# HydrogenSulfate/LFT

Hardware: AMD Instinct MI355X
Metric: LF patches/sec (5x5 angRes, 32x32 LR, 4xSR) (higher is better)
Workload: dtype bf16; 1 GPU; LFT 5x5 angRes 4xSR inference, batch=4 per GPU, 32x32 LR patches; global_batch=4, parallelism=dp1 (independent shards), streams_per_gpu=1, hip_graph=True, steps_in_flight=2

## Files before the change

### lft_amd/_lib.py

```python
from __future__ import annotations

import ctypes
import os
import subprocess
from ctypes import POINTER, c_char_p, c_float, c_int, c_longlong, c_size_t, c_void_p

HERE = os.path.dirname(os.path.abspath(__file__))
CSRC = os.path.join(HERE, "csrc")
LIB_PATH = os.environ.get("LFT_LIB_PATH") or os.path.join(HERE, "liblft_hip.so")
SOURCES = ["lft_api.hip", "lft_common.cuh", "lft_kernels_a.cuh", "lft_kernels_b.cuh", "lft_train.cuh", "lft_train_host.cuh", "lft_metrics.cuh", "lft_prepare.cuh"]
ABI_VERSION = 5
STATUS_NONFINITE = 1001

PREC_F32, PREC_BF16, PREC_F16 = 0, 1, 2
MATH_F32, MATH_BF16X3, MATH_BF16X6 = 0, 1, 2
NUM_PARAMS = 78

_lib = None


class LftError(RuntimeError):
    pass


# ... 73 lines not shown
                                     c_int, POINTER(c_float), POINTER(c_char_p), POINTER(c_int)]),
    "lft_kernel_time": (c_int, [c_char_p, c_void_p, c_void_p, c_int, c_int, c_int, c_int, c_int, c_int, c_int, c_void_p, POINTER(c_float)]),
    "lft_bicubic_fwd": (c_int, [c_void_p, c_void_p, c_int, c_int, c_int, c_int, c_int, c_void_p]),
    "lft_init_features_fwd": (c_int, [c_void_p, c_void_p, c_void_p, c_void_p, c_int, c_int, c_int, c_int, c_int, c_int, c_void_p]),
    "lft_ang_block_fwd": (c_int, [c_void_p, c_int, c_void_p, c_void_p, c_int, c_int, c_int, c_int, c_int, c_int, c_void_p]),
    "lft_spa_block_fwd": (c_int, [c_void_p, c_int, c_void_p, c_void_p, c_void_p, c_void_p, c_int, c_int, c_int, c_int, c_int, c_int, c_void_p]),
    "lft_upsample_fwd": (c_int, [c_void_p, c_void_p, c_void_p, c_void_p, c_void_p, c_int, c_int, c_int, c_int, c_int, c_int, c_void_p]),
    "lft_scene_counts": (c_int, [c_int, c_int, c_int, c_int, POINTER(c_int), POINTER(c_int)]),
    "lft_scene_divide": (c_int, [c_void_p, c_void_p, c_int, c_int, c_int, c_int, c_int, c_void_p]),
    "lft_scene_integrate": (c_int, [c_void_p, c_void_p, c_int, c_int, c_int, c_int, c_int, c_int, c_void_p]),
    "lft_train_tape_bytes": (c_int, [c_int, c_int, c_int, c_int, c_int, POINTER(c_size_t)]),
    "lft_train_grad_floats": (c_int, [c_int, POINTER(c_size_t)]),
    "lft_train_tape_offset": (c_int, [c_char_p, c_int, c_int, c_int, c_int, c_int, POINTER(c_size_t)]),
    "lft_train_forward": (c_int, [POINTER(c_void_p), c_int, c_void_p, c_void_p, c_void_p, c_int, c_int, c_int, c_int, c_int, c_int, c_void_p]),
    "lft_train_backward": (c_int, [POINTER(c_void_p), c_int, c_void_p, c_void_p, c_void_p, c_void_p, c_int, c_int, c_int, c_int, c_int, c_int, c_void_p]),
    "lft_train_backward_input": (c_int, [POINTER(c_void_p), c_int, c_void_p, c_void_p, c_void_p, c_void_p, c_void_p,
                                         c_int, c_int, c_int, c_int, c_int, c_int, c_void_p]),
    "lft_lr_grad_bwd": (c_int, [c_void_p, c_void_p, c_void_p, c_void_p, c_int, c_int, c_int, c_int, c_int, c_void_p]),
    "lft_train_backward_buckets": (c_int, [POINTER(c_void_p), c_int, c_void_p, c_void_p, c_void_p, c_void_p, c_int, c_int, c_int, c_int, c_int, c_int,
                                           c_void_p, c_void_p, c_void_p]),
    "lft_train_block_backward": (c_int, [POINTER(c_void_p), c_int, c_void_p, c_void_p, c_int, c_int, c_void_p, c_void_p, c_void_p,
                                         c_int, c_int, c_int, c_int, c_int, c_int, c_void_p]),
    "lft_train_grad_bucket": (c_int, [c_int, c_int, POINTER(c_size_t), POINTER(c_size_t)]),
    "lft_train_step_profiled": (c_int, [POINTER(c_void_p), c_int, c_void_p, c_void_p, c_void_p, c_void_p, c_void_p, c_int, c_int, c_int, c_int, c_int, c_int,
                                        c_void_p, c_int, POINTER(c_float), POINTER(c_char_p), POINTER(c_int)]),
    "lft_l1_loss": (c_int, [c_void_p, c_void_p, c_longlong, c_void_p, c_float, c_void_p, c_void_p, c_void_p]),
    "lft_adam_step": (c_int, [c_void_p, c_void_p, c_void_p, c_void_p, c_longlong, c_float, c_float, c_float, c_float, c_int, c_float, c_float, c_void_p]),
    "lft_view_metrics_scratch_bytes": (c_int, [c_int, c_int, c_int, c_int, POINTER(c_size_t)]),
    "lft_view_metrics": (c_int, [c_void_p, c_void_p, c_int, c_int, c_int, c_int, c_float, c_void_p, c_void_p, c_void_p, c_void_p]),
    "lft_lf_prepare": (c_int, [c_void_p, c_int, c_int, c_int, c_int, c_int, c_int, POINTER(c_longlong), c_int, c_int,
                               POINTER(c_int), c_int, c_int, c_int, c_void_p, c_void_p, c_int, c_void_p, c_void_p, c_int,
                               c_void_p, c_void_p, c_void_p]),
    "lft_mfma_selftest": (c_int, [c_void_p, c_void_p, c_void_p, c_void_p, c_void_p, c_int, c_void_p]),
}
EXPORTS = tuple(_SIGS)
TEST_EXPORTS = ("lft_mfma_selftest",)
BLOCK_UPSAMPLE, BLOCK_SPA, BLOCK_ANG, BLOCK_INIT = 0, 1, 2, 3
LF_UINT8, LF_FLOAT32, LF_FLOAT64 = 0, 1, 2
GRAD_BUCKETS = 3
BUCKET_FN = ctypes.CFUNCTYPE(c_int, c_void_p, c_int, c_size_t, c_size_t)


def lib() -> ctypes.CDLL:
    global _lib
    if _lib is None:
        if not os.path.exists(LIB_PATH):
            raise LftError(f"{LIB_PATH} is missing: the HIP extension has not been built "
                           "(run __graft_entry__.build()); there is no CPU fallback")
        L = ctypes.CDLL(LIB_PATH)
        L.lft_version.restype, L.lft_version.argtypes = c_int, []
        got = L.lft_version()
        if got != ABI_VERSION:
            raise LftError(f"{LIB_PATH} reports ABI version {got}, this binding needs {ABI_VERSION}: rebuild it (__graft_entry__.build())")
        for name, (res, args) in _SIGS.items():
            fn = getattr(L, name)
            fn.restype, fn.argtypes = res, args
        _lib = L
    return _lib


def check(rc: int, what: str) -> None:
    if rc != 0:
        msg = lib().lft_last_error()
        raise LftError(f"{what} failed (code {rc}): {msg.decode() if msg else ''}")


def packed_bytes(A, h, w, s, prec) -> int:
    n = c_size_t(0)
    check(lib().lft_packed_bytes(A, h, w, s, prec, ctypes.byref(n)), "lft_packed_bytes")
    return n.value


def workspace_bytes(B, A, h, w, s, prec) -> int:
    n = c_size_t(0)
    check(lib().lft_workspace_bytes(B, A, h, w, s, prec, ctypes.byref(n)), "lft_workspace_bytes")
    return n.value
```

### lft_amd/csrc/lft_api.hip

```cpp
#include "../../include/lft_hip.h"
#include "../../include/lft_hip_test.h"
#include <hip/hip_runtime.h>
#include <stdint.h>

#include <cstdarg>
#include <cstdio>
#include <cmath>
#include <set>
#include <string>
#include <algorithm>
#include <type_traits>
#include <utility>
#include <vector>

#ifndef LFT_TU
#define LFT_TU 0
#endif

namespace {
#include "lft_kernels_a.cuh"
#include "lft_kernels_b.cuh"
#include "lft_metrics.cuh"
#include "lft_prepare.cuh"
#include "lft_train.cuh"
// ... 78 lines not shown

template <auto... Vs, typename V, typename F> int dispatch(V v, F&& f) {
    int rc = 0;
    if (((v == Vs && ((rc = f(std::integral_constant<decltype(Vs), Vs>{})), true)) || ...)) return rc;
    return fail(LFT_ERR_ARG, "internal: no kernel variant for %d", (int)v);
}
template <int V> using int_c = std::integral_constant<int, V>;
template <typename F> int by_prec(int prec, F&& f) {
    if (prec == LFT_PREC_F32) return f(float{});
    if (prec == LFT_PREC_BF16) return f(bf16_t{});
    return f(f16_t{});
}
inline size_t align256(size_t x) { return (x + 255) & ~(size_t)255; }

struct Dims {
    int B, A, V, h, w, hw, s, gp, gt, nchunk;
    long long ntok;
};

int make_dims(int B, int A, int h, int w, int s, int prec, Dims* d) {
    if (prec != LFT_PREC_F32 && prec != LFT_PREC_BF16 && prec != LFT_PREC_F16)
        return fail(LFT_ERR_ARG, "prec must be LFT_PREC_F32, LFT_PREC_BF16 or LFT_PREC_F16, got %d", prec);
    if (B < 1 || A < 1 || h < 1 || w < 1) return fail(LFT_ERR_SHAPE, "B, A, h, w must be positive (B=%d A=%d h=%d w=%d)", B, A, h, w);
    if (s != 2 && s != 4) return fail(LFT_ERR_SHAPE, "scale factor must be 2 or 4, got %d", s);
    if (A * A > 128) return fail(LFT_ERR_UNSUPPORTED, "angRes %d (A*A=%d views > 128) is not implemented in this build", A, A * A);
    if ((long long)B * A * A * h * w > (1LL << 27)) return fail(LFT_ERR_SHAPE, "too many tokens");
    d->B = B; d->A = A; d->V = A * A; d->h = h; d->w = w; d->hw = h * w; d->s = s;
    d->gp = (s + 2) * (s + 2); d->gt = (d->gp + 31) / 32; d->nchunk = 2 * s * s;
    d->ntok = (long long)B * d->V * d->hw;
    return 0;
}

constexpr int kFragsConv = 72, kFragsAng = 64, kFragsSpa1 = 240, kFragsSpa1NoQ = 208, kFragsSpa2 = 176;
inline int frags_up(const Dims& d) { return d.nchunk * (4 + 2 * d.gt); }

struct PackedLayout {
    size_t conv0_w, ln_ang[kLayers], ln_spa[kLayers], ang_pe, petok[kLayers], spa_pe_img;
    size_t s_conv[3], s_ang[kLayers], s_spa1[kLayers], s_spa2[kLayers], s_up, total;
};

PackedLayout packed_layout(const Dims& d, int prec) {
    const size_t esz = prec == LFT_PREC_F32 ? 4 : 2, fragb = 64 * 8 * esz;
    PackedLayout L;
    size_t o = 0;
    auto take = [&](size_t bytes) { size_t r = o; o = align256(o + bytes); return r; };
    L.conv0_w = take(576 * 4);
    for (int l = 0; l < kLayers; ++l) { L.ln_ang[l] = take(256 * 4); L.ln_spa[l] = take(512 * 4); }
    L.ang_pe = take((size_t)((d.V + 31) / 32) * 2048 * 4);
    for (int l = 0; l < kLayers; ++l) L.petok[l] = take((size_t)((d.hw + 32 * kNwSpa1 - 1) / (32 * kNwSpa1)) * kNwSpa1 * 4096 * esz);
    L.spa_pe_img = take((size_t)d.hw * 64 * esz);
    for (int i = 0; i < 3; ++i) L.s_conv[i] = take(kFragsConv * fragb);
    for (int l = 0; l < kLayers; ++l) {
        L.s_ang[l] = take(kFragsAng * fragb);
        L.s_spa1[l] = take(kFragsSpa1 * fragb);
        L.s_spa2[l] = take(kFragsSpa2 * fragb);
    }
    L.s_up = take((size_t)frags_up(d) * fragb);
    L.total = o;
    return L;
}

struct WorkLayout {
    size_t x0, feat, xa, xb, tok, q, k, v, o, g, status, total;
};
WorkLayout work_layout(const Dims& d, int prec) {
    const size_t esz = prec == LFT_PREC_F32 ? 4 : 2;
    WorkLayout W;
// ... 119 lines not shown
            std::vector<PackOp> ops;
            ops.push_back(lin_op(q[12], 0, 64, 64, 0, 4, 1, kAngScale));
            ops.push_back(lin_op(q[12], 64, 64, 64, 0, 4, 1, 1.0f));
            ops.push_back(lin_op(q[12], 128, 64, 64, 0, 4, 1, 1.0f));
            ops.push_back(lin_op(q[13], 0, 64, 64, 0, 4, 1, 1.0f));
            ops.push_back(lin_op(q[16], 0, 128, 64, 0, 4, 1, 1.0f));
            ops.push_back(lin_op(q[17], 0, 64, 128, 0, 8, 1, 1.0f));
            if ((rc = run_pack<T>(ops, at<T>(packed, L.s_ang[l]), kFragsAng, st))) return rc;
        }
        {
            std::vector<PackOp> ops;
            conv_ops(ops, q[0], 128);
            ops.push_back(lin_op(q[3], 256, 128, 128, 0, 8, 1, 1.0f));
            ops.push_back(lin_op(q[3], 128, 128, 128, 0, 8, 1, 1.0f));
            ops.push_back(lin_op(q[3], 0, 128, 128, 0, 8, 1, kSpaScale));
            if ((rc = run_pack<T>(ops, at<T>(packed, L.s_spa1[l]), kFragsSpa1, st))) return rc;
        }
        {
            std::vector<PackOp> ops;
            ops.push_back(lin_op(q[4], 0, 128, 128, 0, 8, (sizeof(T) == 2 && tok_lane_major<T>(d)) ? 1 : 0, 1.0f));
            for (int c = 0; c < 4; ++c) {
                ops.push_back(lin_op(q[7], 64 * c, 64, 128, 0, 8, 1, 1.0f));
                ops.push_back(lin_op(q[8], 0, 128, 256, 64 * c, 4, 1, 1.0f));
            }
            ops.push_back(lin_op(q[9], 0, 64, 128, 0, 8, 1, 1.0f));
            if ((rc = run_pack<T>(ops, at<T>(packed, L.s_spa2[l]), kFragsSpa2, st))) return rc;
        }
        if ((rc = launch_spa1<T, true>((unsigned)((d.hw + 32 * kNwSpa1 - 1) / (32 * kNwSpa1)), at<T>(packed, L.spa_pe_img), at<T>(packed, L.s_spa1[l]), nullptr, nullptr,
                                       nullptr, nullptr, nullptr, nullptr, at<T>(packed, L.petok[l]), 1, d, st, nullptr))) return rc;
        LFT_LAUNCH_OK("k_spa1<pe>");
    }
    {
        std::vector<PackOp> ops;
        for (int c = 0; c < d.nchunk; ++c) {
            ops.push_back(lin_op(P[76], 32 * c, 32, 64, 0, 4, 1, 1.0f));
            PackOp m = lin_op(P[77], 0, d.gp, 0, 32 * c, 2, 1, 1.0f);
            m.kind = 1; m.s = d.s; m.ntiles = d.gt;
            ops.push_back(m);
        }
        if ((rc = run_pack<T>(ops, at<T>(packed, L.s_up), frags_up(d), st))) return rc;
    }
    return 0;
}

void launch_assemble(const float* lr, const float* g, float* out, int B, int A, int h, int w, int s, hipStream_t st, int gld = 0, unsigned* status = nullptr) {
    const dim3 tg((unsigned)((A * w + 7) / 8) * (unsigned)((A * h + 7) / 8) * (unsigned)B);
    if (!gld) gld = (s + 2) * (s + 2);
    if (s == 2) k_assemble_t<2><<<tg, 256, 0, st>>>(lr, g, out, B, A, h, w, gld, status);
    else k_assemble_t<4><<<tg, 256, 0, st>>>(lr, g, out, B, A, h, w, gld, status);
}

template <typename T>
int init_features(const void* packed, const PackedLayout& L, const float* lr, T* x0, T* ta, T* tb, T* feat, const Dims& d, hipStream_t st) {
    const int nimg = d.B * d.V, nwg = nimg * ((d.hw + 32 * kNwConv - 1) / (32 * kNwConv));
    const size_t lds = lds_conv64<T>(d.w);
    int rc;
    if ((rc = allow_lds(k_conv64<T, false>, lds, "k_conv64"))) return rc;
    if ((rc = allow_lds(k_conv64<T, true>, lds, "k_conv64"))) return rc;
    k_conv0<T><<<dim3((unsigned)((d.hw + kConv0Tok - 1) / kConv0Tok), (unsigned)nimg), 256, 0, st>>>(lr, at<float>(packed, L.conv0_w), x0, d.B, d.A, d.h, d.w);
    LFT_LAUNCH_OK("k_conv0");
    k_conv64<T, false><<<nwg, 64 * kNwConv, lds, st>>>(x0, ta, nullptr, at<T>(packed, L.s_conv[0]), nimg, d.h, d.w);
    LFT_LAUNCH_OK("k_conv64");
    k_conv64<T, false><<<nwg, 64 * kNwConv, lds, st>>>(ta, tb, nullptr, at<T>(packed, L.s_conv[1]), nimg, d.h, d.w);
    LFT_LAUNCH_OK("k_conv64");
    k_conv64<T, true><<<nwg, 64 * kNwConv, lds, st>>>(tb, feat, x0, at<T>(packed, L.s_conv[2]), nimg, d.h, d.w);
    LFT_LAUNCH_OK("k_conv64");
    return 0;
}
template <typename T, int CT, int LL>
int ang_multi(const void* packed, const PackedLayout& L, int l, const T* in, T* out, const Dims& d, hipStream_t st, unsigned* status) {
    constexpr bool WLDS = sizeof(T) == 2;
    constexpr int NG = (sizeof(T) == 2 && CT <= 3) ? 2 : 1;
    constexpr size_t FB = 1024 * FragInfo<T>::PIECES;
    const size_t lds = (WLDS ? 64 * FB : 0) + 1024 + (size_t)NG * CT * 8 * FB + (size_t)NG * CT * TileIO<2, T>::BYTES;
    const int npix = d.B * d.hw;
    int rc;
    const unsigned grid = std::min<unsigned>(blocks_for(npix, NG), 256u * (unsigned)std::max<size_t>(1, kMaxLds / lds));
    if ((rc = allow_lds(k_ang_multi<T, CT, WLDS, NG, LL>, lds, "k_ang_multi"))) return rc;
    k_ang_multi<T, CT, WLDS, NG, LL><<<grid, 64 * CT * NG, lds, st>>>(in, out, at<T>(packed, L.s_ang[l]), at<float>(packed, L.ln_ang[l]),
                                                                     at<float>(packed, L.ang_pe), d.V, d.hw, npix, status);
    LFT_LAUNCH_OK("k_ang");
    return 0;
}
template <typename T>
int ang_block(const void* packed, const PackedLayout& L, int l, const T* in, T* out, const Dims& d, hipStream_t st, unsigned* status = nullptr) {
    auto multi = [&](auto CT, auto LL) { return ang_multi<T, CT, LL>(packed, L, l, in, out, d, st, status); };
    if (d.V > 100) return multi(int_c<4>{}, int_c<13>{});
    if (d.V > 96) return multi(int_c<4>{}, int_c<9>{});
    if (d.V > 64) return multi(int_c<3>{}, int_c<9>{});
    if (d.V == 64) return multi(int_c<2>{}, int_c<16>{});
    if (d.V > 32) return multi(int_c<2>{}, int_c<9>{});
    const int npix = d.B * d.hw;
    const size_t lds = lds_ang<T>();
    int rc;
    const unsigned grid = std::min<unsigned>(blocks_for(npix, 4), 256u * (unsigned)std::max<size_t>(1, kMaxLds / lds));
// ... 213 lines not shown
int lft_kernel_time(const char* kernel, const void* packed, void* workspace, int B, int A, int h, int w, int s, int prec, int reps,
                    void* stream, float* ms_out) {
    Dims d; int rc;
    if (!kernel || !packed || !workspace || !ms_out || reps < 1) return fail(LFT_ERR_ARG, "bad argument");
    if ((rc = make_dims(B, A, h, w, s, prec, &d))) return rc;
    hipStream_t st = static_cast<hipStream_t>(stream);
    return by_prec(prec, [&](auto t) { using T = decltype(t); return kernel_time_impl<T>(kernel, packed, workspace, d, prec, reps, st, ms_out); });
}

int lft_bicubic_fwd(const float* lr, float* out, int B, int A, int h, int w, int s, void* stream) {
    Dims d; int rc;
    if (!lr || !out) return fail(LFT_ERR_ARG, "null pointer");
    if ((rc = make_dims(B, A, h, w, s, LFT_PREC_F32, &d))) return rc;
    const dim3 grid((unsigned)((A * w * s + 255) / 256), (unsigned)(A * h * s), (unsigned)B);
    k_bicubic<<<grid, 256, 0, static_cast<hipStream_t>(stream)>>>(lr, out, B, A, h, w, s);
    LFT_LAUNCH_OK("k_bicubic");
    return 0;
}

int lft_init_features_fwd(const void* packed, const float* lr, void* act_out, void* workspace, int B, int A, int h, int w, int s,
                          int prec, void* stream) {
    Dims d; int rc;
    if (!packed || !lr || !act_out || !workspace) return fail(LFT_ERR_ARG, "null pointer");
    if ((rc = make_dims(B, A, h, w, s, prec, &d))) return rc;
    const PackedLayout L = packed_layout(d, prec);
    const WorkLayout W = work_layout(d, prec);
    hipStream_t st = static_cast<hipStream_t>(stream);
    return by_prec(prec, [&](auto t) {
        using T = decltype(t);
        return init_features<T>(packed, L, lr, at<T>(workspace, W.x0), at<T>(workspace, W.xa), at<T>(workspace, W.xb), static_cast<T*>(act_out), d, st);
    });
}

int lft_ang_block_fwd(const void* packed, int layer, const void* act_in, void* act_out, int B, int A, int h, int w, int s, int prec,
                      void* stream) {
    Dims d; int rc;
    if (!packed || !act_in || !act_out) return fail(LFT_ERR_ARG, "null pointer");
    if (layer < 0 || layer >= kLayers) return fail(LFT_ERR_ARG, "layer %d out of range", layer);
    if ((rc = make_dims(B, A, h, w, s, prec, &d))) return rc;
    const PackedLayout L = packed_layout(d, prec);
    hipStream_t st = static_cast<hipStream_t>(stream);
    return by_prec(prec, [&](auto t) {
        using T = decltype(t);
        return ang_block<T>(packed, L, layer, static_cast<const T*>(act_in), static_cast<T*>(act_out), d, st);
    });
}

int lft_spa_block_fwd(const void* packed, int layer, const void* act_in, const void* skip, void* act_out, void* workspace, int B, int A,
                      int h, int w, int s, int prec, void* stream) {
    Dims d; int rc;
    if (!packed || !act_in || !act_out || !workspace) return fail(LFT_ERR_ARG, "null pointer");
    if (layer < 0 || layer >= kLayers) return fail(LFT_ERR_ARG, "layer %d out of range", layer);
    if ((rc = make_dims(B, A, h, w, s, prec, &d))) return rc;
    const PackedLayout L = packed_layout(d, prec);
    const WorkLayout W = work_layout(d, prec);
    hipStream_t st = static_cast<hipStream_t>(stream);
    return by_prec(prec, [&](auto t) {
        using T = decltype(t);
        return spa_block<T>(packed, L, layer, static_cast<const T*>(act_in), static_cast<const T*>(skip), static_cast<T*>(act_out), workspace, W, d, st);
    });
}

int lft_upsample_fwd(const void* packed, const void* act_in, const float* lr, float* out, void* workspace, int B, int A, int h, int w,
                     int s, int prec, void* stream) {
    Dims d; int rc;
    if (!packed || !act_in || !lr || !out || !workspace) return fail(LFT_ERR_ARG, "null pointer");
// ... 29 lines not shown
    return 0;
}
int lft_scene_counts(int h0, int w0, int patch, int stride, int* num_u, int* num_v) {
    if (!num_u || !num_v) return fail(LFT_ERR_ARG, "null pointer");
    return scene_counts(h0, w0, patch, stride, num_u, num_v);
}
int lft_scene_divide(const float* scene, float* patches, int A, int h0, int w0, int patch, int stride, void* stream) {
    int nu, nv, rc;
    if (!scene || !patches || A < 1) return fail(LFT_ERR_ARG, "bad argument");
    if ((rc = scene_counts(h0, w0, patch, stride, &nu, &nv))) return rc;
    const dim3 grid((unsigned)((A * patch + 255) / 256), (unsigned)(A * patch), (unsigned)(nu * nv));
    k_scene_divide<<<grid, 256, 0, static_cast<hipStream_t>(stream)>>>(scene, patches, A, h0, w0, patch, stride, nv);
    LFT_LAUNCH_OK("k_scene_divide");
    return 0;
}
int lft_scene_integrate(const float* sr_patches, float* sr_scene, int A, int h0, int w0, int patch, int stride, int s, void* stream) {
    int nu, nv, rc;
    if (!sr_patches || !sr_scene || A < 1 || s < 1) return fail(LFT_ERR_ARG, "bad argument");
    if ((rc = scene_counts(h0, w0, patch, stride, &nu, &nv))) return rc;
    const dim3 grid((unsigned)((A * w0 * s + 255) / 256), (unsigned)(A * h0 * s));
    k_scene_integrate<<<grid, 256, 0, static_cast<hipStream_t>(stream)>>>(sr_patches, sr_scene, A, patch * s, stride * s, h0 * s, w0 * s, nv);
    LFT_LAUNCH_OK("k_scene_integrate");
    return 0;
}

int lft_mfma_selftest(const float* Am, const float* Bm, const float* W2, float* C, float* D, int prec, void* stream) {
    if (!Am || !Bm || !W2 || !C || !D) return fail(LFT_ERR_ARG, "null pointer");
    hipStream_t st = static_cast<hipStream_t>(stream);
    if (prec == LFT_PREC_F32) k_selftest<float><<<1, 64, 0, st>>>(Am, Bm, W2, C, D);
    else if (prec == LFT_PREC_BF16) k_selftest<bf16_t><<<1, 64, 0, st>>>(Am, Bm, W2, C, D);
    else if (prec == LFT_PREC_F16) k_selftest<f16_t><<<1, 64, 0, st>>>(Am, Bm, W2, C, D);
    else return fail(LFT_ERR_ARG, "bad prec %d", prec);
    LFT_LAUNCH_OK("k_selftest");
    return 0;
}

int lft_view_metrics_scratch_bytes(int B, int A, int h, int w, size_t* out_bytes) {
    if (!out_bytes || B < 1 || A < 1 || h < 1 || w < 1) return fail(LFT_ERR_ARG, "bad argument");
    const size_t ntiles = (size_t)((h + kMetTile - 1) / kMetTile) * ((w + kMetTile - 1) / kMetTile);
    *out_bytes = (size_t)B * A * A * ntiles * 3 * sizeof(double);
    return 0;
}
int lft_view_metrics(const float* label, const float* out, int B, int A, int h, int w, float ssim_range, float* psnr, float* ssim,
                     void* scratch, void* stream) {
    if (!label || !out || !psnr || !ssim || !scratch || B < 1 || A < 1) return fail(LFT_ERR_ARG, "bad argument");
    if (h < 11 || w < 11) return fail(LFT_ERR_SHAPE, "views of %dx%d are smaller than the 11x11 SSIM window", h, w);
    hipStream_t st = static_cast<hipStream_t>(stream);
    const int ntiles = ((h + kMetTile - 1) / kMetTile) * ((w + kMetTile - 1) / kMetTile), nviews = B * A * A;
    const double C1 = (0.01 * ssim_range) * (0.01 * ssim_range), C2 = (0.03 * ssim_range) * (0.03 * ssim_range);
    k_view_metrics<<<dim3((unsigned)ntiles, (unsigned)nviews), 256, 0, st>>>(label, out, static_cast<double*>(scratch), A, h, w, C1, C2);
    LFT_LAUNCH_OK("k_view_metrics");
    k_view_metrics_final<<<blocks_for(nviews, 64), 64, 0, st>>>(static_cast<const double*>(scratch), nviews, ntiles, h, w, psnr, ssim);
    LFT_LAUNCH_OK("k_view_metrics_final");
    return 0;
}
int lft_lf_prepare(const void* lf, int lf_class, int U, int V, int H, int W, int C, const long long* strides, int A, int s,
                   const int* crops, int n_crops, int crop_h, int crop_w, const double* weights_h, const int* indices_h, int taps_h,
                   const double* weights_w, const int* indices_w, int taps_w, float* hr, float* lr, void* stream) {
    if (!lf || !strides || !crops || !weights_h || !indices_h || !weights_w || !indices_w || !hr || !lr)
        return fail(LFT_ERR_ARG, "lft_lf_prepare: null pointer");
    if (lf_class != LFT_LF_UINT8 && lf_class != LFT_LF_FLOAT32 && lf_class != LFT_LF_FLOAT64)
        return fail(LFT_ERR_ARG, "lft_lf_prepare: light-field class must be LFT_LF_UINT8, LFT_LF_FLOAT32 or LFT_LF_FLOAT64, got %d", lf_class);
    if (U < 1 || V < 1 || H < 1 || W < 1 || C < 3)
        return fail(LFT_ERR_ARG, "lft_lf_prepare: light field [%d,%d,%d,%d,%d] needs positive sizes and at least 3 channels", U, V, H, W, C);
    for (int i = 0; i < 5; ++i)
        if (strides[i] < 0) return fail(LFT_ERR_ARG, "lft_lf_prepare: stride %d is negative (%lld)", i, strides[i]);
// ... 182 lines not shown
```

### lft_amd/csrc/lft_kernels_a.cuh

```cuda
#pragma once
#include "lft_common.cuh"

struct PackOp {
    const float* src;
    int kind, row0, nrows, ntiles, ld, kmul, kadd, k0, ksteps, kmap, frag0, s;
    float scale;
    int order;
};
__host__ __device__ __forceinline__ int wfrag_index(int OT, int KS, int ot, int ks) {
    const int g = ot >> 2, G = OT - 4 * g < 4 ? OT - 4 * g : 4;
    return 4 * g * KS + ks * G + (ot & 3);
}
__host__ __device__ __forceinline__ void wfrag_coords(int OT, int KS, int lf, int order, int& nt, int& ks) {
    if (!order) { nt = lf / KS; ks = lf % KS; return; }
    const int gl = (OT - 1) >> 2, g = lf / (4 * KS) < gl ? lf / (4 * KS) : gl, G = OT - 4 * g < 4 ? OT - 4 * g : 4, rem = lf - 4 * g * KS;
    ks = rem / G; nt = 4 * g + rem % G;
}
constexpr int LFT_PACK_MAXOPS = 40;
struct PackArgs {
    int nops;
    PackOp op[LFT_PACK_MAXOPS];
};

LFT_DEV float upm_entry(const float* __restrict__ w3, int n, int kk, int s) {
    const int I = n / (s + 2) - 1, J = n % (s + 2) - 1;
    const int c = kk / (s * s), i = (kk / s) % s, j = kk % s;
    const int dy = i - I, dx = j - J;
    if (dy < -1 || dy > 1 || dx < -1 || dx > 1) return 0.0f;
    return w3[c * 9 + (dy + 1) * 3 + (dx + 1)];
}

template <typename T>
__global__ __launch_bounds__(64) void k_pack(PackArgs args, T* __restrict__ dst) {
    const int f = blockIdx.x, lane = threadIdx.x, r = lane & 31, h = lane >> 5;
    int oi = 0;
    for (int i = 0; i < args.nops; ++i)
        if (f >= args.op[i].frag0) oi = i;
    const PackOp& op = args.op[oi];
    int nt, ks;
    wfrag_coords(op.ntiles, op.ksteps, f - op.frag0, op.order, nt, ks);
    const int n = 32 * nt + r;
#pragma unroll
    for (int j = 0; j < 8; ++j) {
        const int kk = op.k0 + 16 * ks + (op.kmap ? 8 * (j >> 2) + 4 * h + (j & 3) : 8 * h + j);
        float v = 0.0f;
        if (n < op.nrows) {
            if (op.kind == 0) v = op.scale * op.src[(size_t)(op.row0 + n) * op.ld + kk * op.kmul + op.kadd];
            else if (op.kind == 1) v = upm_entry(op.src, n, kk, op.s);
            else v = kk < (op.s + 2) * (op.s + 2) ? upm_entry(op.src, kk, n, op.s) : 0.0f;
        }
        if constexpr (sizeof(T) == 4) dst[(((size_t)f * 2 + (j >> 2)) * 64 + lane) * 4 + (j & 3)] = (T)v;
        else dst[((size_t)f * 64 + lane) * 8 + j] = (T)v;
    }
}

LFT_DEV float pe_value(int l, int c) {
    const int m = c & 31;
    const float g = (float)pow(10000.0, (double)(2 * m) / 64.0);
    const float p = (float)l / g;
    return (c < 32) ? (float)sin((double)p) : (float)cos((double)p);
}
template <typename T>
__global__ void k_pe_tables(float* __restrict__ ang_pe, T* __restrict__ spa_img, int V, int h, int w) {
    const int idx = blockIdx.x * blockDim.x + threadIdx.x;
    const int ntile = (V + 31) / 32;
    if (idx < ntile * 2048) {
        const int e = idx & 7, lane = (idx >> 3) & 63, k = (idx >> 9) & 3, ct = idx >> 11;
        const int view = ct * 32 + (lane & 31), nt = k >> 1, g = 2 * (k & 1) + (e >> 2);
        const int ch = 32 * nt + 8 * g + 4 * (lane >> 5) + (e & 3);
        ang_pe[idx] = view < V ? pe_value(view, ch) : 0.0f;
    }
    if (idx < h * w * 64) {
        const int p = idx >> 6, c = idx & 63;
        spa_img[idx] = (T)((pe_value(p / w, c) + pe_value(p % w, c)) / 2.0f);
    }
}
__global__ void k_copy_f32(const float* __restrict__ src, float* __restrict__ dst, int n) {
    const int i = blockIdx.x * blockDim.x + threadIdx.x;
    if (i < n) dst[i] = src[i];
}

// ... 96 lines not shown

constexpr int kConvZeroRow = 256;
LFT_DEV void clear_zero_row(char* zero_row) {
    if (threadIdx.x < kConvZeroRow / 16) store_raw16(zero_row + threadIdx.x * 16, raw16{0u, 0u, 0u, 0u});
}
template <int NT, typename T, int NW, typename Ring>
LFT_DEV void conv3x3_tile(const char* lds_in, const char* zero_row, int tl, int y, int x, bool ok, int h, int w, int hh,
                          Ring& ring, f32x16 (&acc)[NT]) {
    using CI = ConvIn<T, NW>;
    static_assert(CI::ROW_BYTES <= kConvZeroRow, "zero row too short");
#pragma unroll
    for (int tap = 0; tap < 9; ++tap) {
        const int dy = tap / 3 - 1, dx = tap % 3 - 1;
        const int yy = y + dy, xx = x + dx;
        const bool inb = ok && yy >= 0 && yy < h && xx >= 0 && xx < w;
        const int slot = tl + w + 1 + dy * w + dx;
        const char* row = inb ? lds_in + slot * CI::ROW_BYTES : zero_row;
        const int sw = inb ? CI::swz(slot) : 0;
#pragma unroll
        for (int ks = 0; ks < 4; ++ks) {
            Frag<T> b;
            if constexpr (sizeof(T) == 2) {
                b.v = __builtin_bit_cast(typename H16<T>::v8, load_raw16(row + (((2 * ks + hh) ^ sw) * 16)));
            } else {
                b.lo = __builtin_bit_cast(f32x4, load_raw16(row + (((4 * ks + 2 * hh) ^ sw) * 16)));
                b.hi = __builtin_bit_cast(f32x4, load_raw16(row + (((4 * ks + 2 * hh + 1) ^ sw) * 16)));
            }
#pragma unroll
            for (int nt = 0; nt < NT; ++nt) mma(ring.next(), b, acc[nt]);
        }
    }
}

constexpr int kNwConv = 4;
constexpr int kConv64Chunk = 12;
template <typename T, bool RES, int NW = kNwConv>
__global__ __launch_bounds__(64 * NW) void k_conv64(const T* __restrict__ in, T* __restrict__ out, const T* __restrict__ res,
                                                   const T* __restrict__ wstream, int nimg, int h, int w) {
    extern __shared__ __attribute__((aligned(16))) char smem[];
    constexpr int TT = 32 * NW;
    const int lane = threadIdx.x & 63, r = lane & 31, hh = lane >> 5, wave = threadIdx.x >> 6;
    const int hw = h * w, tpi = (hw + TT - 1) / TT;
    const int bid = xcd_tile(blockIdx.x, gridDim.x);
    const int im = bid / tpi, p0 = (bid % tpi) * TT;
    const int tl = wave * 32 + r, p = p0 + tl;
    const bool ok = p < hw;
    const int t0 = p0 + wave * 32, nvalid = max(0, min(32, hw - t0));
    const size_t tile_off = ((size_t)im * hw + min(t0, hw - 1)) * 64;
    char* lds_in = smem + WRing<T, kConv64Chunk, NW>::LDS_BYTES;
    char* scr = lds_in + ConvIn<T, NW>::bytes(w) + wave * TileIO<2, T>::BYTES;
    char* zero_row = lds_in + ConvIn<T, NW>::bytes(w) + NW * TileIO<2, T>::BYTES;
    f32x16 rr[2];
    if (RES) load_tile<2, T>(res + tile_off, nvalid, lane, rr, scr);
    WRing<T, kConv64Chunk, NW> ring;
    ring.init(wstream, smem, 72);
    stage_conv_input<T, NW>(in + (size_t)im * hw * 64, p0, hw, w, lds_in);
    clear_zero_row(zero_row);
    wait_staged();
    __syncthreads();
    LFT_NOTE_ASM_("USE", kNoteConvIn, 0);
    f32x16 acc[2];
    zero_acc<2>(acc);
    conv3x3_tile<2, T, NW>(lds_in, zero_row, tl, p / w, p % w, ok, h, w, hh, ring, acc);
#pragma unroll
    for (int nt = 0; nt < 2; ++nt)
#pragma unroll
        for (int i = 0; i < 16; ++i) acc[nt][i] = lrelu02_fast(acc[nt][i]);
    if (RES) {
#pragma unroll
        for (int nt = 0; nt < 2; ++nt) acc[nt] += rr[nt];
    }
    store_tile<2, T>(out + tile_off, nvalid, lane, acc, scr);
}

template <int NT_OUT, int KS, typename T>
LFT_DEV void linear_lds(const char* wl, int f0, int lane, const Frag<T> (&x)[KS], f32x16 (&y)[NT_OUT]) {
#pragma unroll
    for (int nt = 0; nt < NT_OUT; ++nt)
#pragma unroll
        for (int ks = 0; ks < KS; ++ks)
            mma(frag_from_pieces(wl + (f0 + nt * KS + ks) * 1024 * FragInfo<T>::PIECES, lane, T()), x[ks], y[nt]);
}

template <typename T, int NLIVE = 16>
__global__ __launch_bounds__(256, 2) void k_ang(const T* __restrict__ X, T* __restrict__ Y, const T* __restrict__ ws,
                                             const float* __restrict__ ln, const float* __restrict__ pe,
                                             int V, int hw, int npix, unsigned* __restrict__ status) {
    extern __shared__ __attribute__((aligned(16))) char smem[];
    constexpr int FB = 1024 * FragInfo<T>::PIECES;
    const int lane = threadIdx.x & 63, r = lane & 31, hh = lane >> 5;
    const int wave = __builtin_amdgcn_readfirstlane(threadIdx.x >> 6);
    unsigned bad = 0;
    {
// ... 268 lines not shown
```

### lft_amd/csrc/lft_kernels_b.cuh

```cuda
#pragma once
#include "lft_common.cuh"
#include "lft_kernels_a.cuh"

constexpr int kUpChunk = 8;
constexpr int kSpaChunk = 16;
constexpr int kSpaOcc = 2;
constexpr int kNwSpa1 = 4, kNwSpa2 = 4, kNwUp = 8;
template <typename T, bool PE_ONLY, int CH = kSpaChunk, bool TOKLM = false, bool WITH_Q = true, int NW = kNwSpa1>
__global__ __launch_bounds__(64 * NW, kSpaOcc) void k_spa1(const T* __restrict__ X, const T* __restrict__ ws,
                                              const float* __restrict__ ln, const T* __restrict__ petok,
                                              T* __restrict__ TOK, T* __restrict__ Q, T* __restrict__ K, T* __restrict__ Vv,
                                              T* __restrict__ pe_out, int nimg, int h, int w, unsigned* __restrict__ status) {
    extern __shared__ __attribute__((aligned(16))) char smem[];
    const int lane = threadIdx.x & 63, r = lane & 31, hh = lane >> 5, wave = threadIdx.x >> 6;
    constexpr int TT = 32 * NW;
    const int hw = h * w, tpi = (hw + TT - 1) / TT;
    const int bid = xcd_tile(blockIdx.x, gridDim.x);
    const int im = bid / tpi, p0 = (bid % tpi) * TT;
    const int tl = wave * 32 + r, p = p0 + tl;
    const bool ok = p < hw;
    LFT_STAMP(0);
    typename RawPiece<T>::type pe_raw[16];
    if (!PE_ONLY) load_lane_major_raw<4, T>(petok + (size_t)((p0 >> 5) + wave) * 4096, lane, pe_raw);
    char* lds_in = smem + WRing<T, CH, NW>::LDS_BYTES;
// ... 467 lines not shown
    ffn_chunk(std::integral_constant<int, 2>());
    ffn_chunk(std::integral_constant<int, 3>());
    LFT_STAMP(28);
    acc_frags<4, T>(t, f);
    f32x16 y[2];
    zero_acc<2>(y);
    linear_ring_at<160, 2, 8>(ring, f, y);
    LFT_STAMP(29);
    BlkRows ry = rows; ry.img_row_bytes = w * 128; ry.tok_bytes = 128;
    if (SKIP) {
        f32x16 sk[2];
        load_tile_map<2, T>(skip + tok0 * 64, ry, lane, sk, scr);
#pragma unroll
        for (int nt = 0; nt < 2; ++nt) y[nt] += sk[nt];
    }
    if constexpr (YLM) {
        if (qy < h) {
            T* dst = Y + (img0 + (long long)qy * w + x0) * 64 + (32 * hh + bxl + qpx) * 8;
#pragma unroll
            for (int kidx = 0; kidx < 4; ++kidx) {
                V8 v;
#pragma unroll
                for (int j = 0; j < 8; ++j) v[j] = (T)y[kidx >> 1][8 * (kidx & 1) + j];
                store_raw16(reinterpret_cast<char*>(dst + kidx * 512), __builtin_bit_cast(raw16, v));
            }
        }
    } else {
        store_tile_map<2, T>(Y + tok0 * 64, ry, lane, y, scr);
    }
    LFT_STAMP(30);
    publish_status(status, bad);
}

template <typename T, int GT, bool XLM = false, int NW = kNwUp>
__global__ __launch_bounds__(64 * NW) void k_up(const T* __restrict__ X, const T* __restrict__ ws, float* __restrict__ G,
                                            long long ntok, int nchunk, int gp) {
    extern __shared__ __attribute__((aligned(16))) char smem[];
    const int lane = threadIdx.x & 63, r = lane & 31, hh = lane >> 5;
    const long long tok_raw = ((long long)blockIdx.x * NW + (threadIdx.x >> 6)) * 32 + r;
    const bool ok = tok_raw < ntok;
    const long long tok = ok ? tok_raw : ntok - 1;
    const long long t0 = tok_raw - r;
    const int nvalid = (int)max(0LL, min(32LL, ntok - t0));
    char* scr = smem + WRing<T, kUpChunk, NW>::LDS_BYTES + (threadIdx.x >> 6) * TileIO<2, T>::BYTES;
    WRing<T, kUpChunk, NW> ring;
    ring.init(ws, smem, nchunk * (4 + 2 * GT));
    f32x16 x[2];
    if constexpr (XLM) load_tile_lm<2, T>(X + t0 * 64, lane, x);
    else load_tile<2, T>(X + min(t0, ntok - 1) * 64, nvalid, lane, x, scr);
    Frag<T> xf[4];
    acc_frags<2, T>(x, xf);
    f32x16 g[GT];
    zero_acc<GT>(g);
#pragma unroll 2
    for (int c = 0; c < nchunk; ++c) {
        f32x16 u[1];
        zero_acc<1>(u);
        linear_ring<1, 4, T>(ring, xf, u);
#pragma unroll
        for (int i = 0; i < 16; ++i) u[0][i] = lrelu02_fast(u[0][i]);
        Frag<T> uf[2];
        acc_frags<1, T>(u, uf);
        linear_ring<GT, 2, T>(ring, uf, g);
    }
    if (!ok) return;
#pragma unroll
    for (int nt = 0; nt < GT; ++nt)
#pragma unroll
        for (int grp = 0; grp < 4; ++grp) {
            const int base = 32 * nt + 8 * grp + 4 * hh;
            if (base < gp)
                store4(G + tok * gp + base, f32x4{g[nt][4 * grp], g[nt][4 * grp + 1], g[nt][4 * grp + 2], g[nt][4 * grp + 3]});
        }
}

LFT_DEV void cubic_coef(float t, float (&c)[4]) {
    const float A = -0.75f;
    const float x0 = t + 1.0f, x1 = t, x2 = 1.0f - t, x3 = 2.0f - t;
    c[0] = ((A * x0 - 5.0f * A) * x0 + 8.0f * A) * x0 - 4.0f * A;
    c[1] = ((A + 2.0f) * x1 - (A + 3.0f)) * x1 * x1 + 1.0f;
    c[2] = ((A + 2.0f) * x2 - (A + 3.0f)) * x2 * x2 + 1.0f;
    c[3] = ((A * x3 - 5.0f * A) * x3 + 8.0f * A) * x3 - 4.0f * A;
}
LFT_DEV float bicubic_at(const float* __restrict__ view, int stride, int h, int w, int Y, int X, int s) {
    const float sy = ((float)Y + 0.5f) / (float)s - 0.5f, sx = ((float)X + 0.5f) / (float)s - 0.5f;
    const float fy = floorf(sy), fx = floorf(sx);
    float cy[4], cx[4];
    cubic_coef(sy - fy, cy);
    cubic_coef(sx - fx, cx);
    const int iy = (int)fy, ix = (int)fx;
    float acc = 0.0f;
#pragma unroll
    for (int a = 0; a < 4; ++a) {
        const int yy = min(max(iy - 1 + a, 0), h - 1);
        float row = 0.0f;
#pragma unroll
// ... 178 lines not shown
```

Baseline: 9800 patches/s.

## Exploit upsample-matrix sparsity for 4x SR and fold conv0 into first conv64

```diff
diff --git a/lft_amd/_lib.py b/lft_amd/_lib.py
--- a/lft_amd/_lib.py
+++ b/lft_amd/_lib.py
@@ -129,9 +129,11 @@
                                POINTER(c_int), c_int, c_int, c_int, c_void_p, c_void_p, c_int, c_void_p, c_void_p, c_int,
                                c_void_p, c_void_p, c_void_p]),
     "lft_mfma_selftest": (c_int, [c_void_p, c_void_p, c_void_p, c_void_p, c_void_p, c_int, c_void_p]),
+    "lft_up4_chunk_map": (c_int, [c_int, c_int, POINTER(c_int), POINTER(c_int)]),
+    "lft_init_features_unfused_fwd": (c_int, [c_void_p, c_void_p, c_void_p, c_void_p, c_int, c_int, c_int, c_int, c_int, c_int, c_void_p]),
 }
 EXPORTS = tuple(_SIGS)
-TEST_EXPORTS = ("lft_mfma_selftest",)
+TEST_EXPORTS = ("lft_mfma_selftest", "lft_up4_chunk_map", "lft_init_features_unfused_fwd")
 BLOCK_UPSAMPLE, BLOCK_SPA, BLOCK_ANG, BLOCK_INIT = 0, 1, 2, 3
 LF_UINT8, LF_FLOAT32, LF_FLOAT64 = 0, 1, 2
 GRAD_BUCKETS = 3
@@ -150,6 +152,8 @@
         if got != ABI_VERSION:
             raise LftError(f"{LIB_PATH} reports ABI version {got}, this binding needs {ABI_VERSION}: rebuild it (__graft_entry__.build())")
         for name, (res, args) in _SIGS.items():
+            if name in TEST_EXPORTS and not hasattr(L, name):
+                continue
             fn = getattr(L, name)
             fn.restype, fn.argtypes = res, args
         _lib = L
diff --git a/lft_amd/csrc/lft_api.hip b/lft_amd/csrc/lft_api.hip
--- a/lft_amd/csrc/lft_api.hip
+++ b/lft_amd/csrc/lft_api.hip
@@ -134,7 +134,7 @@
 }
 
 constexpr int kFragsConv = 72, kFragsAng = 64, kFragsSpa1 = 240, kFragsSpa1NoQ = 208, kFragsSpa2 = 176;
-inline int frags_up(const Dims& d) { return d.nchunk * (4 + 2 * d.gt); }
+inline int frags_up(const Dims& d) { return d.nchunk * (4 + 2 * (d.s == 4 ? 1 : d.gt)); }
 
 struct PackedLayout {
     size_t conv0_w, ln_ang[kLayers], ln_spa[kLayers], ang_pe, petok[kLayers], spa_pe_img;
@@ -320,7 +320,15 @@
     }
     {
         std::vector<PackOp> ops;
-        for (int c = 0; c < d.nchunk; ++c) {
+        for (int c = 0; d.s == 4 && c < kUp4Chunks; ++c) {
+            PackOp u = lin_op(P[76], 0, 32, 64, 0, 4, 1, 1.0f);
+            u.upc = c + 1;
+            ops.push_back(u);
+            PackOp m = lin_op(P[77], up4_chunk_row0(c), d.gp - up4_chunk_row0(c), 0, 0, 2, 1, 1.0f);
+            m.kind = 1; m.s = d.s; m.ntiles = 1; m.upc = c + 1;
+            ops.push_back(m);
+        }
+        for (int c = 0; d.s != 4 && c < d.nchunk; ++c) {
             ops.push_back(lin_op(P[76], 32 * c, 32, 64, 0, 4, 1, 1.0f));
             PackOp m = lin_op(P[77], 0, d.gp, 0, 32 * c, 2, 1, 1.0f);
             m.kind = 1; m.s = d.s; m.ntiles = d.gt;
@@ -339,16 +347,24 @@
 }
 
 template <typename T>
-int init_features(const void* packed, const PackedLayout& L, const float* lr, T* x0, T* ta, T* tb, T* feat, const Dims& d, hipStream_t st) {
+int init_features(const void* packed, const PackedLayout& L, const float* lr, T* x0, T* ta, T* tb, T* feat, const Dims& d, hipStream_t st,
+                  bool fold = true) {
     const int nimg = d.B * d.V, nwg = nimg * ((d.hw + 32 * kNwConv - 1) / (32 * kNwConv));
     const size_t lds = lds_conv64<T>(d.w);
     int rc;
     if ((rc = allow_lds(k_conv64<T, false>, lds, "k_conv64"))) return rc;
     if ((rc = allow_lds(k_conv64<T, true>, lds, "k_conv64"))) return rc;
-    k_conv0<T><<<dim3((unsigned)((d.hw + kConv0Tok - 1) / kConv0Tok), (unsigned)nimg), 256, 0, st>>>(lr, at<float>(packed, L.conv0_w), x0, d.B, d.A, d.h, d.w);
-    LFT_LAUNCH_OK("k_conv0");
-    k_conv64<T, false><<<nwg, 64 * kNwConv, lds, st>>>(x0, ta, nullptr, at<T>(packed, L.s_conv[0]), nimg, d.h, d.w);
-    LFT_LAUNCH_OK("k_conv64");
+    if (fold && (size_t)conv0_tile_bytes<kNwConv>(d.w) <= kNwConv * TileIO<2, T>::BYTES) {
+        if ((rc = allow_lds(k_conv64<T, false, true>, lds, "k_conv64"))) return rc;
+        k_conv64<T, false, true><<<nwg, 64 * kNwConv, lds, st>>>(nullptr, ta, nullptr, at<T>(packed, L.s_conv[0]), nimg, d.h, d.w,
+                                                                 lr, at<float>(packed, L.conv0_w), x0, d.A);
+        LFT_LAUNCH_OK("k_conv64");
+    } else {
+        k_conv0<T><<<dim3((unsigned)((d.hw + kConv0Tok - 1) / kConv0Tok), (unsigned)nimg), 256, 0, st>>>(lr, at<float>(packed, L.conv0_w), x0, d.B, d.A, d.h, d.w);
+        LFT_LAUNCH_OK("k_conv0");
+        k_conv64<T, false><<<nwg, 64 * kNwConv, lds, st>>>(x0, ta, nullptr, at<T>(packed, L.s_conv[0]), nimg, d.h, d.w);
+        LFT_LAUNCH_OK("k_conv64");
+    }
     k_conv64<T, false><<<nwg, 64 * kNwConv, lds, st>>>(ta, tb, nullptr, at<T>(packed, L.s_conv[1]), nimg, d.h, d.w);
     LFT_LAUNCH_OK("k_conv64");
     k_conv64<T, true><<<nwg, 64 * kNwConv, lds, st>>>(tb, feat, x0, at<T>(packed, L.s_conv[2]), nimg, d.h, d.w);
@@ -628,6 +644,20 @@
     });
 }
 
+int lft_init_features_unfused_fwd(const void* packed, const float* lr, void* act_out, void* workspace, int B, int A, int h, int w, int s,
+                                  int prec, void* stream) {
+    Dims d; int rc;
+    if (!packed || !lr || !act_out || !workspace) return fail(LFT_ERR_ARG, "null pointer");
+    if ((rc = make_dims(B, A, h, w, s, prec, &d))) return rc;
+    const PackedLayout L = packed_layout(d, prec);
+    const WorkLayout W = work_layout(d, prec);
+    hipStream_t st = static_cast<hipStream_t>(stream);
+    return by_prec(prec, [&](auto t) {
+        using T = decltype(t);
+        return init_features<T>(packed, L, lr, at<T>(workspace, W.x0), at<T>(workspace, W.xa), at<T>(workspace, W.xb), static_cast<T*>(act_out), d, st, false);
+    });
+}
+
 int lft_ang_block_fwd(const void* packed, int layer, const void* act_in, void* act_out, int B, int A, int h, int w, int s, int prec,
                       void* stream) {
     Dims d; int rc;
@@ -723,6 +753,13 @@
     else if (prec == LFT_PREC_F16) k_selftest<f16_t><<<1, 64, 0, st>>>(Am, Bm, W2, C, D);
     else return fail(LFT_ERR_ARG, "bad prec %d", prec);
     LFT_LAUNCH_OK("k_selftest");
+    return 0;
+}
+
+int lft_up4_chunk_map(int chunk, int l, int* channel, int* row0) {
+    if (!channel || !row0 || chunk < 0 || chunk >= kUp4Chunks || l < 0 || l >= 32) return fail(LFT_ERR_ARG, "bad argument");
+    *channel = up4_chunk_channel(chunk, l);
+    *row0 = up4_chunk_row0(chunk);
     return 0;
 }
 
diff --git a/lft_amd/csrc/lft_kernels_a.cuh b/lft_amd/csrc/lft_kernels_a.cuh
--- a/lft_amd/csrc/lft_kernels_a.cuh
+++ b/lft_amd/csrc/lft_kernels_a.cuh
@@ -6,7 +6,11 @@
     int kind, row0, nrows, ntiles, ld, kmul, kadd, k0, ksteps, kmap, frag0, s;
     float scale;
     int order;
+    int upc;
 };
+constexpr int kUp4Chunks = 32, kUp4ChunksLo = 24;
+__host__ __device__ __forceinline__ int up4_chunk_channel(int q, int l) { return (8 * (q & 7) + (l >> 2)) * 16 + 4 * (q >> 3) + (l & 3); }
+__host__ __device__ __forceinline__ int up4_chunk_row0(int q) { return q < kUp4ChunksLo ? 0 : 16; }
 __host__ __device__ __forceinline__ int wfrag_index(int OT, int KS, int ot, int ks) {
     const int g = ot >> 2, G = OT - 4 * g < 4 ? OT - 4 * g : 4;
     return 4 * g * KS + ks * G + (ot & 3);
@@ -45,8 +49,8 @@
         const int kk = op.k0 + 16 * ks + (op.kmap ? 8 * (j >> 2) + 4 * h + (j & 3) : 8 * h + j);
         float v = 0.0f;
         if (n < op.nrows) {
-            if (op.kind == 0) v = op.scale * op.src[(size_t)(op.row0 + n) * op.ld + kk * op.kmul + op.kadd];
-            else if (op.kind == 1) v = upm_entry(op.src, n, kk, op.s);
+            if (op.kind == 0) v = op.scale * op.src[(size_t)(op.upc ? up4_chunk_channel(op.upc - 1, n) : op.row0 + n) * op.ld + kk * op.kmul + op.kadd];
+            else if (op.kind == 1) v = upm_entry(op.src, op.row0 + n, op.upc ? up4_chunk_channel(op.upc - 1, kk) : kk, op.s);
             else v = kk < (op.s + 2) * (op.s + 2) ? upm_entry(op.src, kk, n, op.s) : 0.0f;
         }
         if constexpr (sizeof(T) == 4) dst[(((size_t)f * 2 + (j >> 2)) * 64 + lane) * 4 + (j & 3)] = (T)v;
@@ -209,11 +213,65 @@
     }
 }
 
+template <int NW> __host__ __device__ constexpr int conv0_tile_bytes(int w) { return ((32 * NW + 2 * w + 1) / w + 4) * (w + 2) * 4; }
+template <typename T, int NW>
+LFT_DEV void conv0_into_tile(const float* __restrict__ img, int stride, const float* __restrict__ w0, T* __restrict__ x0_out,
+                             int p0, int h, int w, char* lds_in, float* lrt) {
+    using CI = ConvIn<T, NW>;
+    const int hw = h * w, cg = threadIdx.x & 7, pitch = w + 2;
+    f32x4 wq[18];
+#pragma unroll
+    for (int k = 0; k < 18; ++k) wq[k] = load4(w0 + 72 * cg + 4 * k);
+    const int qlo = max(p0 - w - 1, 0), qhi = min(p0 + 32 * NW + w, hw - 1);
+    const int ylo = qlo / w - 1, nrows = qhi / w + 1 - ylo + 1;
+    for (int i = threadIdx.x; i < nrows * pitch; i += 64 * NW) {
+        const int yy = ylo + i / pitch, xx = i % pitch - 1;
+        const float v = img[min(max(yy, 0), h - 1) * stride + min(max(xx, 0), w - 1)];
+        lrt[i] = (yy >= 0 && yy < h && xx >= 0 && xx < w) ? v : 0.0f;
+    }
+    __syncthreads();
+    for (int s = threadIdx.x >> 3; s < CI::slots(w); s += 8 * NW) {
+        const int q = p0 - w - 1 + s;
+        if (q < 0 || q >= hw) continue;
+        const int y = q / w, x = q - y * w;
+        const float* t0 = lrt + (y - 1 - ylo) * pitch + x;
+        float val[9];
+#pragma unroll
+        for (int t = 0; t < 9; ++t) val[t] = t0[(t / 3) * pitch + t % 3];
+        float o[8];
+#pragma unroll
+        for (int c = 0; c < 8; ++c) {
+            float a = 0.0f;
+#pragma unroll
+            for (int t = 0; t < 9; ++t) a += wq[(9 * c + t) >> 2][(9 * c + t) & 3] * val[t];
+            o[c] = a;
+        }
+        char* row = lds_in + s * CI::ROW_BYTES;
+        const bool own = s >= w + 1 && s < w + 1 + 32 * NW;
+        T* grow = x0_out + (size_t)q * 64 + cg * 8;
+        if constexpr (sizeof(T) == 2) {
+            typename H16<T>::v8 v;
+#pragma unroll
+            for (int c = 0; c < 8; ++c) v[c] = (T)o[c];
+            store_raw16(row + ((cg ^ CI::swz(s)) * 16), __builtin_bit_cast(raw16, v));
+            if (own) store_raw16(reinterpret_cast<char*>(grow), __builtin_bit_cast(raw16, v));
+        } else {
+            const f32x4 lo{o[0], o[1], o[2], o[3]}, hi{o[4], o[5], o[6], o[7]};
+            store_raw16(row + (((2 * cg) ^ CI::swz(s)) * 16), __builtin_bit_cast(raw16, lo));
+            store_raw16(row + (((2 * cg + 1) ^ CI::swz(s)) * 16), __builtin_bit_cast(raw16, hi));
+            if (own) { store4(grow, lo); store4(grow + 4, hi); }
+        }
+    }
+}
+
 constexpr int kNwConv = 4;
 constexpr int kConv64Chunk = 12;
-template <typename T, bool RES, int NW = kNwConv>
+template <typename T, bool RES, bool X0 = false, int NW = kNwConv>
 __global__ __launch_bounds__(64 * NW) void k_conv64(const T* __restrict__ in, T* __restrict__ out, const T* __restrict__ res,
-                                                   const T* __restrict__ wstream, int nimg, int h, int w) {
+                                                   const T* __restrict__ wstream, int nimg, int h, int w,
+                                                   const float* __restrict__ lr = nullptr, const float* __restrict__ w0 = nullptr,
+                                                   T* __restrict__ x0_out = nullptr, int A = 1) {
+    static_assert(!(RES && X0), "conv_init0 is folded into the first conv_init only");
     extern __shared__ __attribute__((aligned(16))) char smem[];
     constexpr int TT = 32 * NW;
     const int lane = threadIdx.x & 63, r = lane & 31, hh = lane >> 5, wave = threadIdx.x >> 6;
@@ -231,11 +289,21 @@
     if (RES) load_tile<2, T>(res + tile_off, nvalid, lane, rr, scr);
     WRing<T, kConv64Chunk, NW> ring;
     ring.init(wstream, smem, 72);
-    stage_conv_input<T, NW>(in + (size_t)im * hw * 64, p0, hw, w, lds_in);
-    clear_zero_row(zero_row);
-    wait_staged();
-    __syncthreads();
-    LFT_NOTE_ASM_("USE", kNoteConvIn, 0);
+    if constexpr (X0) {
+        const int V = A * A, b = im / V, v = im - b * V, a1 = v / A, a2 = v - a1 * A;
+        const float* img = lr + (size_t)b * (A * h) * (A * w) + (size_t)(a1 * h) * (A * w) + a2 * w;
+        conv0_into_tile<T, NW>(img, A * w, w0, x0_out + (size_t)im * hw * 64, p0, h, w, lds_in,
+                               reinterpret_cast<float*>(lds_in + ConvIn<T, NW>::bytes(w)));
+        clear_zero_row(zero_row);
+        wait_staged();
+        __syncthreads();
+    } else {
+        stage_conv_input<T, NW>(in + (size_t)im * hw * 64, p0, hw, w, lds_in);
+        clear_zero_row(zero_row);
+        wait_staged();
+        __syncthreads();
+        LFT_NOTE_ASM_("USE", kNoteConvIn, 0);
+    }
     f32x16 acc[2];
     zero_acc<2>(acc);
     conv3x3_tile<2, T, NW>(lds_in, zero_row, tl, p / w, p % w, ok, h, w, hh, ring, acc);
diff --git a/lft_amd/csrc/lft_kernels_b.cuh b/lft_amd/csrc/lft_kernels_b.cuh
--- a/lft_amd/csrc/lft_kernels_b.cuh
+++ b/lft_amd/csrc/lft_kernels_b.cuh
@@ -523,6 +523,17 @@
     publish_status(status, bad);
 }
 
+template <typename T, int NW>
+LFT_DEV void up_chunk(WRing<T, kUpChunk, NW>& ring, const Frag<T> (&xf)[4], f32x16 (&g)[1]) {
+    f32x16 u[1];
+    zero_acc<1>(u);
+    linear_ring<1, 4, T>(ring, xf, u);
+#pragma unroll
+    for (int i = 0; i < 16; ++i) u[0][i] = lrelu02_fast(u[0][i]);
+    Frag<T> uf[2];
+    acc_frags<1, T>(u, uf);
+    linear_ring<1, 2, T>(ring, uf, g);
+}
 template <typename T, int GT, bool XLM = false, int NW = kNwUp>
 __global__ __launch_bounds__(64 * NW) void k_up(const T* __restrict__ X, const T* __restrict__ ws, float* __restrict__ G,
                                             long long ntok, int nchunk, int gp) {
@@ -535,7 +546,7 @@
     const int nvalid = (int)max(0LL, min(32LL, ntok - t0));
     char* scr = smem + WRing<T, kUpChunk, NW>::LDS_BYTES + (threadIdx.x >> 6) * TileIO<2, T>::BYTES;
     WRing<T, kUpChunk, NW> ring;
-    ring.init(ws, smem, nchunk * (4 + 2 * GT));
+    ring.init(ws, smem, GT == 2 ? kUp4Chunks * 6 : nchunk * 6);
     f32x16 x[2];
     if constexpr (XLM) load_tile_lm<2, T>(X + t0 * 64, lane, x);
     else load_tile<2, T>(X + min(t0, ntok - 1) * 64, nvalid, lane, x, scr);
@@ -543,16 +554,22 @@
     acc_frags<2, T>(x, xf);
     f32x16 g[GT];
     zero_acc<GT>(g);
+    if constexpr (GT == 2) {
+        f32x16 g0[1], g1[1];
+        zero_acc<1>(g0);
+        zero_acc<1>(g1);
+#pragma unroll
+        for (int c = 0; c < kUp4ChunksLo; ++c) up_chunk(ring, xf, g0);
+#pragma unroll
+        for (int c = kUp4ChunksLo; c < kUp4Chunks; ++c) up_chunk(ring, xf, g1);
+        g[0] = g0[0];
+#pragma unroll
+        for (int e = 0; e < 8; ++e) g[0][e + 8] += g1[0][e];
+#pragma unroll
+        for (int e = 0; e < 4; ++e) g[GT - 1][e] = g1[0][8 + e];
+    } else {
 #pragma unroll 2
-    for (int c = 0; c < nchunk; ++c) {
-        f32x16 u[1];
-        zero_acc<1>(u);
-        linear_ring<1, 4, T>(ring, xf, u);
-#pragma unroll
-        for (int i = 0; i < 16; ++i) u[0][i] = lrelu02_fast(u[0][i]);
-        Frag<T> uf[2];
-        acc_frags<1, T>(u, uf);
-        linear_ring<GT, 2, T>(ring, uf, g);
+        for (int c = 0; c < nchunk; ++c) up_chunk(ring, xf, g);
     }
     if (!ok) return;
 #pragma unroll
```

After: 9988 patches/s (median of 6 runs). 1.02x the previous value.
